# liwanyue123/SRBD-NMPC-Solver

Measured on AMD Instinct MI355X. Metric: SRBD OCP-QP solves/sec (N=20, nx=12, nu=12, fp64) at 1/2/4/8 MI355X, higher is better.
Workload: dtype f64

## Files before the change

srbd-nmpc-solver_amd/csrc/riccati_unconstr_impl.h:

```cpp
namespace srbd {
namespace SRBD_NS {

using real = SRBD_REAL;


struct HbmSrc {
  const ProblemArgsT<real>& a;
  int qp;
  __device__ const real* at(const real* base, int nstage, int blk, int k) const {
    return a.layout == 1 ? base + ((size_t)k * a.batch + qp) * blk
                         : base + ((size_t)qp * nstage + k) * blk;
  }
  __device__ const real* A(int k) const { return at(a.A, a.N, 144, k); }
  __device__ const real* B(int k) const { return at(a.B, a.N, 144, k); }
  __device__ const real* b(int k) const { return at(a.b, a.N, 12, k); }
  __device__ const real* Q(int k) const { return at(a.Q, a.N + 1, 144, k); }
  __device__ const real* S(int k) const { return at(a.S, a.N, 144, k); }
  __device__ const real* R(int k) const { return at(a.R, a.N, 144, k); }
  __device__ const real* q(int k) const { return at(a.q, a.N + 1, 12, k); }
  __device__ const real* r(int k) const { return at(a.r, a.N, 12, k); }
  __device__ real* rec(int k) const { return a.ws + ((size_t)k * a.batch + qp) * kWsStage; }
  real* img = nullptr;
  int gq = 0;
  __device__ real* kept(int k) const { return img + (k * 4 + gq) * kWsStage; }
  template <class StoreRec>
  __device__ void store_stage(int k, StoreRec&& store) const;
};

template <class Src>
constexpr bool keeps_turnaround = std::is_same_v<Src, HbmSrc> && sizeof(real) == 8;

constexpr int kImgA = 0, kImgB = 144, kImgb = 288, kImgQ = 300, kImgS = 444, kImgR = 588,
              kImgq = 732, kImgr = 744, kImgStage = 756, kImgRec = kImgQ;
static_assert(kImgRec + kWsStage <= kImgStage, "a record fits its stage slot past A, B, b");

struct LdsSrc {
  real* img;
  real* grec = nullptr;
  int batch = 0, qp = 0;
  __device__ real* slot(int k) const { return img + k * kImgStage; }
  __device__ const real* A(int k) const { return slot(k) + kImgA; }
  __device__ const real* B(int k) const { return slot(k) + kImgB; }
  __device__ const real* b(int k) const { return slot(k) + kImgb; }
  __device__ const real* Q(int k) const { return slot(k) + kImgQ; }
  __device__ const real* S(int k) const { return slot(k) + kImgS; }
  __device__ const real* R(int k) const { return slot(k) + kImgR; }
  __device__ const real* q(int k) const { return slot(k) + kImgq; }
  __device__ const real* r(int k) const { return slot(k) + kImgr; }
  __device__ real* rec(int k) const {
    return grec ? grec + ((size_t)k * batch + qp) * kWsStage : slot(k) + kImgRec;
  }
};

__device__ __forceinline__ void store_rec_P(real* rec, int lane, const real (&P)[12]) {
  if (lane < kMaxDim) store_packed_col(rec + kWsP, lane, P);
  if (lane == kVecLane) store12(rec + kWsp, P);
}
__device__ __forceinline__ void store_rec(real* rec, int lane, const real (&Kc)[12], const real (&P)[12]) {
  const bool isv = lane == kVecLane;
  if (lane < kMaxDim || isv) {
    const int c = isv ? kMaxDim : lane;
    sfor<0, 12>([&](auto m) {
      constexpr int M = decltype(m)::value;
      rec[kWsK + M * kWsRow + c] = Kc[M];
    });
  }
  store_rec_P(rec, lane, P);
}

constexpr int kRecHotStages = 4;

template <class StoreRec>
__device__ void HbmSrc::store_stage(int k, StoreRec&& store) const {
  if (!img) {
    store(rec(k));
    return;
  }
  if (k < 2) {
    store(kept(k));
    lds_wave_fence();
    return;
  }
  store(img + gq * kWsStage);
  lds_wave_fence();
  const int qp0 = qp - gq;
  const int nq = a.batch - qp0 < 4 ? a.batch - qp0 : 4;
  constexpr int kPiecesPerRec = kWsStage * (int)sizeof(real) / 16;
  const int pieces = nq * kPiecesPerRec;
  typedef double d2 __attribute__((ext_vector_type(2)));
  const d2* src = reinterpret_cast<const d2*>(img);
  d2* dst = reinterpret_cast<d2*>(a.ws + ((size_t)k * a.batch + qp0) * kWsStage);
  const int l = (int)(threadIdx.x & 63);
  if (k >= kRecHotStages) {
    for (int p = l; p < pieces; p += 16 * nq) __builtin_nontemporal_store(src[p], &dst[p]);
  } else {
    for (int p = l; p < pieces; p += 16 * nq) dst[p] = src[p];
  }
  lds_wave_fence();
}

__device__ __forceinline__ void store_riccati_out(const ProblemArgsT<real>& a, int qp, int k, int lane,
                                                  const real (&F)[12], const real (&Kc)[12]) {
  const int N = a.N;
  const bool own = lane < kMaxDim, isv = lane == kVecLane;
  if (a.P && own) store12(a.P + ((size_t)qp * (N + 1) + k) * 144 + (size_t)lane * 12, F);
  if (a.p && isv) store12(a.p + ((size_t)qp * (N + 1) + k) * 12, F);
  if (k < N) {
    if (a.K && own) store12(a.K + ((size_t)qp * N + k) * 144 + (size_t)lane * 12, Kc);
    if (a.k && isv) store12(a.k + ((size_t)qp * N + k) * 12, Kc);
  }
}

constexpr int kLineVec = 4 * 4 * 12;
constexpr int kLineOut = 0;
constexpr int kLineB = 3 * kLineVec;
constexpr int kLinePieces = 4 * 12 * (int)sizeof(real) / 16;
static_assert(kLineB + 2 * kLineVec <= 4 * kWsStage, "the line staging fits slot A");
#ifndef SRBD_RIC_FLUSH_NT
#define SRBD_RIC_FLUSH_NT 1
#endif

template <class Src>
__device__ __forceinline__ void fwd_sweep(const ProblemArgsT<real>& a, const Src& src, const int qp,
                                          const int lane, real* so = nullptr) {
  constexpr int nx = 12, nu = 12;
  const int N = a.N;
  const bool own = lane < kMaxDim;
  const int row = own ? lane : kMaxDim - 1;
  real xv = own ? a.x0[(size_t)qp * nx + lane] : real(0.0);
  bool bad = false;
  real* xo = a.x + (size_t)qp * (N + 1) * nx;
  real* uo = a.u + (size_t)qp * N * nu;
  real* po = a.pi + (size_t)qp * (N + 1) * nx;
  real Pr[12], Kr[12], Ar[12], pv, kv, bv;
  typedef double d2 __attribute__((ext_vector_type(2)));
  typedef __attribute__((address_space(3))) real lds_real;
  typedef __attribute__((address_space(3))) d2 lds_d2;
  lds_real* line = nullptr;
  int gq = 0, qp0 = qp, nq = 1, wl = 0;
  if constexpr (keeps_turnaround<Src>) {
    line = (lds_real*)(uintptr_t)__builtin_amdgcn_readfirstlane((unsigned)(uintptr_t)(lds_real*)src.img);
    gq = src.gq;
    qp0 = __builtin_amdgcn_readfirstlane(qp - gq);
    nq = a.batch - qp0 < 4 ? a.batch - qp0 : 4;
    wl = (int)(threadIdx.x & 63);
  }
  auto piece = [&](int l, int i, int& g, int& w) {
    const int p = l + i * 16 * nq;
    g = p / kLinePieces;
    w = p - g * kLinePieces;
    return p < nq * kLinePieces;
  };
  auto fetch_b = [&](int c) {
    int l = wl;
    opaque(l);
    lds_d2* dst = (lds_d2*)(line + kLineB + (c & 1) * kLineVec);
    d2 bq[2];
    sfor<0, 2>([&](auto i) {
      constexpr int I = decltype(i)::value;
      int g, w;
      bq[I] = d2{0.0, 0.0};
      if (piece(l, I, g, w) && 4 * c + w / 6 < N) {
        const HbmSrc o{a, qp0 + g};
        bq[I] = reinterpret_cast<const d2*>(o.b(4 * c + w / 6))[w % 6];
      }
    });
    sfor<0, 2>([&](auto i) {
      constexpr int I = decltype(i)::value;
      int g, w;
      if (piece(l, I, g, w)) dst[l + I * 16 * nq] = bq[I];
    });
    lds_wave_fence();
  };
  auto flush_out = [&](int c) {
    lds_wave_fence();
    int l = wl;
    opaque(l);
    sfor<0, 2>([&](auto i) {
      constexpr int I = decltype(i)::value;
      int g, w;
      const bool live = piece(l, I, g, w);
      sfor<0, 3>([&](auto v) {
        constexpr int V = decltype(v)::value;
        const int rows = V == 1 ? N : N + 1;
        real* base = V == 0 ? a.x : V == 1 ? a.u : a.pi;
        const int left = rows - 4 * c, nr = left < 4 ? left : 4;
        const lds_d2* from = (const lds_d2*)(line + kLineOut + V * kLineVec);
        if (live && w < 6 * nr) {
          d2* to = reinterpret_cast<d2*>(base + ((size_t)(qp0 + g) * rows + 4 * c) * 12) + w;
          if constexpr (SRBD_RIC_FLUSH_NT) {
            __builtin_nontemporal_store(from[l + I * 16 * nq], to);
          } else {
            *to = from[l + I * 16 * nq];
          }
        }
      });
    });
    lds_wave_fence();
  };
  auto load_rows = [&](int k, real (&P_)[12], real (&K_)[12], real (&A__)[12], real& p_, real& k_,
                       real& b_) {
    const real* rec = src.rec(k);
    load_packed_sym(rec + kWsP, row, P_);
    p_ = rec[kWsp + row];
    if (k < N) {
      const real* kr = rec + kWsK + row * kWsRow;
      const real* Ab = src.A(k);
      sfor<0, 12>([&](auto j) {
        constexpr int J = decltype(j)::value;
        K_[J] = kr[J];
        A__[J] = Ab[J * 12 + row];
      });
      k_ = kr[12];
      if constexpr (keeps_turnaround<Src>) {
        b_ = line[kLineB + ((k >> 2) & 1) * kLineVec + (gq * 4 + (k & 3)) * 12 + row];
      } else {
        b_ = src.b(k)[row];
      }
    }
  };
  auto load_rows_kept = [&](int k, real (&P_)[12], real (&K_)[12], real (&A__)[12], real& p_, real& k_,
                            real& b_) {
    if constexpr (keeps_turnaround<Src>) {
      const auto rec = (const __attribute__((address_space(3))) real*)src.kept(k);
      load_packed_sym(rec + kWsP, row, P_);
      p_ = rec[kWsp + row];
      const auto kr = rec + kWsK + row * kWsRow;
      const real* Ab = src.A(k);
      sfor<0, 12>([&](auto j) {
        constexpr int J = decltype(j)::value;
        K_[J] = kr[J];
        A__[J] = Ab[J * 12 + row];
      });
      k_ = kr[12];
      b_ = src.b(k)[row];
    }
  };
  auto kept = [&](int k) { return keeps_turnaround<Src> && k < 2 && k < N; };
  if (kept(0)) {
    load_rows_kept(0, Pr, Kr, Ar, pv, kv, bv);
    lds_wave_fence();
  } else {
    load_rows(0, Pr, Kr, Ar, pv, kv, bv);
  }
#pragma unroll 1
  for (int k = 0; k <= N; ++k) {
    real Br[12];
    if (k < N) {
      const real* Bb = src.B(k);
      sfor<0, 12>([&](auto j) { Br[decltype(j)::value] = Bb[decltype(j)::value * 12 + row]; });
    }
    const int fc = k == 0 ? 0 : (k >> 2) + 1;
    const bool fetch = keeps_turnaround<Src> && (k == 0 || (k & 3) == 1) && 4 * fc < N;
    real Pn[12], Kn[12], An[12], pvn = real(0.0), kvn = real(0.0), bvn = real(0.0);
    if (k < N) {
      if (kept(k + 1)) {
        load_rows_kept(k + 1, Pn, Kn, An, pvn, kvn, bvn);
      } else {
        load_rows(k + 1, Pn, Kn, An, pvn, kvn, bvn);
      }
    }
    real bx[12];
    sfor<0, 12>([&](auto j) {
      constexpr int J = decltype(j)::value;
      bx[J] = bc<J>(xv);
    });
    real pp = pv;
    sfor<0, 12>([&](auto j) {
      constexpr int J = decltype(j)::value;
      pp = fmadd(Pr[J], bx[J], pp);
    });
    if (own) {
      if constexpr (keeps_turnaround<Src>) {
        line[kLineOut + (gq * 4 + (k & 3)) * 12 + lane] = xv;
        line[kLineOut + 2 * kLineVec + (gq * 4 + (k & 3)) * 12 + lane] = pp;
      } else {
        xo[(size_t)k * nx + lane] = xv;
        po[(size_t)k * nx + lane] = pp;
      }
      if (so) {
        so[k * nx + lane] = xv;
        so[(2 * N + 1) * nx + k * nx + lane] = pp;
      }
    }
    if (k == N) break;
    real uu = kv, xn = bv;
    sfor<0, 12>([&](auto j) {
      constexpr int J = decltype(j)::value;
      uu = fmadd(Kr[J], bx[J], uu);
      xn = fmadd(Ar[J], bx[J], xn);
    });
    if (own) {
      if constexpr (keeps_turnaround<Src>) {
        line[kLineOut + kLineVec + (gq * 4 + (k & 3)) * 12 + lane] = uu;
      } else {
        uo[(size_t)k * nu + lane] = uu;
      }
      if (so) so[(N + 1) * nx + k * nu + lane] = uu;
    }
    xn = dot_bcast(Br, uu, xn);
    bad |= own && (!(uu == uu) || !(xn == xn));
    xv = xn;
    sfor<0, 12>([&](auto j) {
      constexpr int J = decltype(j)::value;
      Pr[J] = Pn[J];
      Kr[J] = Kn[J];
      Ar[J] = An[J];
    });
    pv = pvn;
    kv = kvn;
    bv = bvn;
    if constexpr (keeps_turnaround<Src>) {
      if ((k & 3) == 3) flush_out(k >> 2);
      if (fetch) fetch_b(fc);
    }
  }
  if constexpr (keeps_turnaround<Src>) flush_out(N >> 2);
  if (a.status || a.iter) {
    const unsigned long long m = __ballot(bad);
    const int shift = (threadIdx.x & 63) & ~(kGroup - 1);
    const bool any_bad = ((m >> shift) & 0xffffull) != 0;
    if (lane == 0) {
      if (a.status) a.status[qp] = any_bad ? 3 : 0;
      if (a.iter) a.iter[qp] = 0;
    }
  }
}

template <bool SQRT, class Src>
__device__ __forceinline__ void solve_qp(const ProblemArgsT<real>& a, const Src& src, const int qp,
                                         const int lane, real* so = nullptr) {
  const int N = a.N;
  const bool isv = lane == kVecLane;
  const bool own = lane < kMaxDim;
  const int col = own ? lane : kMaxDim - 1;
  const real reg = a.reg;

  real P[12];
  if (isv) {
    load12(src.q(N), P);
  } else {
    load12(src.Q(N) + col * 12, P);
  }
  store_rec_P(src.rec(N), lane, P);
  store_riccati_out(a, qp, N, lane, P, P);
  if constexpr (SQRT) sqrt_factor(P, lane);

  real A_[12], B_[12];
#pragma unroll 1
  for (int k = N - 1; k >= 0; --k) {
    if (isv) {
      load12(src.b(k), A_);
      sfor<0, 12>([&](auto i) { B_[decltype(i)::value] = real(0.0); });
    } else {
      load12(src.A(k) + col * 12, A_);
      load12(src.B(k) + col * 12, B_);
    }
    auto loadR = [&](real (&Rc)[12]) {
      if (isv) {
        sfor<0, 12>([&](auto i) { Rc[decltype(i)::value] = real(0.0); });
      } else {
        load12(src.R(k) + col * 12, Rc);
      }
    };
    auto loadSQ = [&](real (&Sc)[12], real (&Qc)[12]) {
      if (isv) {
        load12(src.r(k), Sc);
        load12(src.q(k), Qc);
      } else {
        load12(src.S(k) + col * 12, Sc);
        load12(src.Q(k) + col * 12, Qc);
      }
    };
    StageFactor<real> f;
    tstamp(0);
    if constexpr (SQRT) {
      riccati_step_sqrt<1, false>(P, A_, B_, loadR, loadSQ, lane, reg, f);
    } else {
      riccati_step<1, false>(P, A_, B_, loadR, loadSQ, lane, reg, f);
    }
    if constexpr (std::is_same_v<Src, HbmSrc>) {
      src.store_stage(k, [&](real* r) { store_rec(r, lane, f.Kc, f.F); });
    } else {
      store_rec(src.rec(k), lane, f.Kc, f.F);
    }
    tstamp(11);
    store_riccati_out(a, qp, k, lane, f.F, f.Kc);
    sfor<0, 12>([&](auto i) {
      constexpr int I = decltype(i)::value;
      P[I] = f.F[I];
    });
    if constexpr (SQRT) sqrt_factor(P, lane);
  }
  tstamp(12);
  fwd_sweep(a, src, qp, lane, so);
  tstamp(13);
}

template <bool SQRT>
__global__ void __launch_bounds__(256, 2) riccati_unconstr_kernel(ProblemArgsT<real> a) {
  const int gid = blockIdx.x * blockDim.x + threadIdx.x;
  const int qp = gid >> 4;
  if (qp >= a.batch) return;
  if constexpr (sizeof(real) == 8) {
    __shared__ __attribute__((aligned(16))) real rec_img[4 * 2 * 4 * kWsStage];
    static_assert(sizeof(rec_img) <= 64 * 1024, "static LDS limit");
    HbmSrc src{a, qp};
    src.gq = (threadIdx.x >> 4) & 3;
    src.img = rec_img + (threadIdx.x >> 6) * 2 * 4 * kWsStage;
    solve_qp<SQRT>(a, src, qp, threadIdx.x & (kGroup - 1));
  } else {
    solve_qp<SQRT>(a, HbmSrc{a, qp}, qp, threadIdx.x & (kGroup - 1));
  }
}

constexpr int kRealsPerDma = 16 / (int)sizeof(real);
constexpr int kLdsCopyThreads = 512;

__device__ __forceinline__ const real* img_source(const ProblemArgsT<real>& a, int qp, int e) {
  const int N = a.N;
  const int k = e / kImgStage, o = e - k * kImgStage;
  const size_t s = (size_t)qp * N + k, s1 = (size_t)qp * (N + 1) + k;
  if (o >= kImgQ && o < kImgS) return a.Q + s1 * 144 + (o - kImgQ);
  if (o >= kImgq && o < kImgr) return a.q + s1 * 12 + (o - kImgq);
  if (k >= N) return nullptr;
  if (o < kImgB) return a.A + s * 144 + o;
  if (o < kImgb) return a.B + s * 144 + (o - kImgB);
  if (o < kImgQ) return a.b + s * 12 + (o - kImgb);
  if (o < kImgR) return a.S + s * 144 + (o - kImgS);
  if (o < kImgq) return a.R + s * 144 + (o - kImgR);
  return a.r + s * 12 + (o - kImgr);
}

__device__ __forceinline__ void lds_copy_range(const ProblemArgsT<real>& a, real* img, int qp, int e0, int e1,
                                               int t, int nthr) {
  const int wave_off = (t >> 6) * 64 * kRealsPerDma;
  for (int c0 = e0; c0 < e1; c0 += nthr * kRealsPerDma) {
    const int e = c0 + t * kRealsPerDma;
    const real* g = e < e1 ? img_source(a, qp, e) : nullptr;
    if (g)
      __builtin_amdgcn_global_load_lds((const __attribute__((address_space(1))) void*)g,
                                       (__attribute__((address_space(3))) void*)(img + c0 + wave_off), 16,
                                       0, 0);
  }
}
__device__ __forceinline__ void lds_copy_qp(const ProblemArgsT<real>& a, real* img, int qp) {
  lds_copy_range(a, img, qp, 0, (a.N + 1) * kImgStage, threadIdx.x, kLdsCopyThreads);
  tstamp(14);
  asm volatile("s_waitcnt vmcnt(0)" ::: "memory");
  __syncthreads();
  tstamp(15);
}

template <bool SQRT>
__global__ void __launch_bounds__(kLdsCopyThreads, 1) riccati_unconstr_lds_kernel(ProblemArgsT<real> a) {
  extern __shared__ __attribute__((aligned(16))) unsigned char lds_raw[];
  real* img = reinterpret_cast<real*>(lds_raw);
  const int qp = blockIdx.x;
  tstamp(16);
  lds_copy_qp(a, img, qp);
  if (threadIdx.x >= kGroup) return;
  solve_qp<SQRT>(a, LdsSrc{img}, qp, threadIdx.x);
}

size_t lds_image_bytes(int N) { return (size_t)(N + 1) * kImgStage * sizeof(real); }
size_t lds_res_bytes(int N) { return lds_image_bytes(N) + (size_t)(3 * N + 2) * 12 * sizeof(real); }


constexpr int kResThreads = 256;
constexpr int kResStages = kResThreads / 12;
constexpr int kResWavesMax = 8;

__device__ __forceinline__ void max_nan(real& m, real v) {
  v = v < real(0) ? -v : v;
  if (v > m || v != v) m = v;
}

struct ResGlobal {
  const ProblemArgsT<real>& a;
  int qp;
  __device__ const real* at(const real* base, int nstage, size_t blk, int k) const {
    return a.layout == 1 ? base + ((size_t)k * a.batch + qp) * blk : base + ((size_t)qp * nstage + k) * blk;
  }
  __device__ const real* A(int k) const { return at(a.A, a.N, (size_t)a.nx * a.nx, k); }
  __device__ const real* B(int k) const { return at(a.B, a.N, (size_t)a.nx * a.nu, k); }
  __device__ const real* b(int k) const { return at(a.b, a.N, a.nx, k); }
  __device__ const real* Q(int k) const { return at(a.Q, a.N + 1, (size_t)a.nx * a.nx, k); }
  __device__ const real* S(int k) const { return at(a.S, a.N, (size_t)a.nx * a.nu, k); }
  __device__ const real* R(int k) const { return at(a.R, a.N, (size_t)a.nu * a.nu, k); }
  __device__ const real* q(int k) const { return at(a.q, a.N + 1, a.nx, k); }
  __device__ const real* r(int k) const { return at(a.r, a.N, a.nu, k); }
  __device__ const real* x() const { return a.x + (size_t)qp * (a.N + 1) * a.nx; }
  __device__ const real* u() const { return a.u + (size_t)qp * a.N * a.nu; }
  __device__ const real* pi() const { return a.pi + (size_t)qp * (a.N + 1) * a.nx; }
};
struct ResLds : LdsSrc {
  const real* so;
  int N;
  __device__ const real* x() const { return so; }
  __device__ const real* u() const { return so + (N + 1) * 12; }
  __device__ const real* pi() const { return so + (2 * N + 1) * 12; }
};

template <class Acc, int DIM = 0>
__device__ __forceinline__ void unconstr_residuals_body(const ProblemArgsT<real>& a, const Acc& acc, int qp, int t) {
  const int N = a.N, nx = DIM ? DIM : a.nx, nu = DIM ? DIM : a.nu;
  if (a.stat) {
    real* tab = a.stat + (size_t)qp * a.stat_rows * kStatCols;
    for (int i = t; i < a.stat_rows * kStatCols; i += blockDim.x) tab[i] = real(0);
  }
  const real* x = acc.x();
  const real* u = acc.u();
  const real* pi = acc.pi();
  const int i = t % 12;
  real mg = real(0), mb = real(0), ob = real(0);
  for (int k = t / 12; t < kResStages * 12 && k <= N; k += kResStages) {
    const real* xk = x + (size_t)k * nx;
    if (k < N) {
      const real* uk = u + (size_t)k * nu;
      const real* xn = x + (size_t)(k + 1) * nx;
      const real* pn = pi + (size_t)(k + 1) * nx;
      const real* A = acc.A(k);
      const real* B = acc.B(k);
      if (i < nu) {
        const real* S = acc.S(k);
        const real* R = acc.R(k);
        const real* r = acc.r(k);
        real ru = real(0), sx = real(0), bp = real(0);
        for (int j = 0; j < nu; ++j) ru += R[(size_t)j * nu + i] * uk[j];
        for (int j = 0; j < nx; ++j) sx += S[(size_t)j * nu + i] * xk[j];
        for (int j = 0; j < nx; ++j) bp += B[(size_t)i * nx + j] * pn[j];
        max_nan(mg, ru + sx + r[i] + bp);
        ob += uk[i] * (real(0.5) * ru + r[i] + sx);
      }
      if (i < nx) {
        const real* b = acc.b(k);
        real v = b[i] - xn[i];
        for (int j = 0; j < nx; ++j) v += A[(size_t)j * nx + i] * xk[j];
        for (int j = 0; j < nu; ++j) v += B[(size_t)j * nx + i] * uk[j];
        max_nan(mb, v);
      }
    }
    if (k > 0 && i < nx) {
      const real* Q = acc.Q(k);
      const real* q = acc.q(k);
      real qx = real(0), g = q[i] - pi[(size_t)k * nx + i];
      for (int j = 0; j < nx; ++j) qx += Q[(size_t)j * nx + i] * xk[j];
      g += qx;
      if (k < N) {
        const real* uk = u + (size_t)k * nu;
        const real* pn = pi + (size_t)(k + 1) * nx;
        const real* A = acc.A(k);
        const real* S = acc.S(k);
        for (int j = 0; j < nu; ++j) g += S[(size_t)i * nu + j] * uk[j];
        for (int j = 0; j < nx; ++j) g += A[(size_t)i * nx + j] * pn[j];
      }
      max_nan(mg, g);
      ob += xk[i] * (real(0.5) * qx + q[i]);
    }
  }
  for (int m = 32; m >= 1; m >>= 1) {
    const real og = __shfl_xor(mg, m), obb = __shfl_xor(mb, m);
    if (og > mg || og != og) mg = og;
    if (obb > mb || obb != obb) mb = obb;
    ob += __shfl_xor(ob, m);
  }
  __shared__ real part[3][kResWavesMax];
  const int w = t / 64;
  if ((t & 63) == 0) {
    part[0][w] = mg;
    part[1][w] = mb;
    part[2][w] = ob;
  }
  __syncthreads();
  if (t == 0) {
    mg = part[0][0], mb = part[1][0], ob = part[2][0];
    for (int j = 1; j < kResThreads / 64; ++j) {
      if (part[0][j] > mg || part[0][j] != part[0][j]) mg = part[0][j];
      if (part[1][j] > mb || part[1][j] != part[1][j]) mb = part[1][j];
      ob += part[2][j];
    }
    if (a.res) {
      a.res[(size_t)qp * 4 + 0] = mg;
      a.res[(size_t)qp * 4 + 1] = mb;
      a.res[(size_t)qp * 4 + 2] = real(0);
      a.res[(size_t)qp * 4 + 3] = real(0);
    }
    if (a.obj) a.obj[qp] = ob;
    if (a.stat) {
      real* row = a.stat + (size_t)qp * a.stat_rows * kStatCols;
      row[6] = mg;
      row[7] = mb;
      row[10] = ob;
    }
    if (a.status && (mg != mg || mb != mb)) a.status[qp] = 3;
  }
}

__global__ void __launch_bounds__(kResThreads) unconstr_residuals_kernel(ProblemArgsT<real> a) {
  unconstr_residuals_body(a, ResGlobal{a, (int)blockIdx.x}, (int)blockIdx.x, (int)threadIdx.x);
}

template <bool SQRT>
__global__ void __launch_bounds__(kLdsCopyThreads, 1) riccati_unconstr_lds_res_kernel(ProblemArgsT<real> a) {
  extern __shared__ __attribute__((aligned(16))) unsigned char lds_raw[];
  real* img = reinterpret_cast<real*>(lds_raw);
  real* so = img + (a.N + 1) * kImgStage;
  const int qp = blockIdx.x;
  tstamp(16);
  lds_copy_qp(a, img, qp);
  LdsSrc src{img};
  src.grec = a.ws;
  src.batch = a.batch;
  src.qp = qp;
  if (threadIdx.x < kGroup) solve_qp<SQRT>(a, src, qp, threadIdx.x, so);
  __syncthreads();
  ResLds acc{};
  acc.img = img;
  acc.so = so;
  acc.N = a.N;
  unconstr_residuals_body(a, acc, qp, (int)threadIdx.x);
}

template <bool FULL>
__global__ void __launch_bounds__(256) unconstr_residuals_group_kernel(ProblemArgsT<real> a) {
  __shared__ __attribute__((aligned(16))) real tb_all[(256 / kGroup) * 144];
  const int qp = (int)((blockIdx.x * blockDim.x + threadIdx.x) >> 4);
  const int lane = threadIdx.x & (kGroup - 1);
  if (qp >= a.batch) return;
  real* const tb = tb_all + (threadIdx.x >> 4) * 144;
  const int N = a.N, nx = FULL ? 12 : a.nx, nu = FULL ? 12 : a.nu;
  if (a.stat) {
    real* tab = a.stat + (size_t)qp * a.stat_rows * kStatCols;
    for (int i = lane; i < a.stat_rows * kStatCols; i += kGroup) tab[i] = real(0);
  }
  const bool smaj = a.layout == 1;
  auto at = [&](const real* base, int nstage, size_t blk, int k) -> const real* {
    return smaj ? base + ((size_t)k * a.batch + qp) * blk : base + ((size_t)qp * nstage + k) * blk;
  };
  const size_t nxx = (size_t)nx * nx, nxu = (size_t)nx * nu, nuu = (size_t)nu * nu;
  const real* x = a.x + (size_t)qp * (N + 1) * nx;
  const real* u = a.u + (size_t)qp * N * nu;
  const real* pi = a.pi + (size_t)qp * (N + 1) * nx;
  const int li = lane < kMaxDim ? lane : 0;
  const bool xl = lane < nx, ul = lane < nu;
  auto colv = [&](const real* blk, int rows, int cols, real (&v)[12]) {
    if constexpr (FULL) {
      load12(blk + li * 12, v);
    } else {
      load_col_pad(blk + (size_t)li * rows, rows, lane < cols, v);
    }
  };
  auto row_sum = [&](const real (&T)[12]) -> real {
    lds_wave_fence();
    if (lane < kMaxDim) store12(tb + lane * 12, T);
    lds_wave_fence();
    real s = real(0);
    sfor<0, 12>([&](auto j) { s += tb[decltype(j)::value * 12 + li]; });
    return s;
  };
  real mg = real(0), mb = real(0), ob = real(0);
#pragma unroll 1
  for (int k = 0; k <= N; ++k) {
    const real xk = xl ? x[(size_t)k * nx + lane] : real(0);
    real T[12];
    real gx = real(0);
    if (k > 0) {
      real Qc[12];
      colv(at(a.Q, N + 1, nxx, k), nx, nx, Qc);
      sfor<0, 12>([&](auto i) { T[decltype(i)::value] = Qc[decltype(i)::value] * xk; });
      const real qx = row_sum(T);
      const real qk = xl ? at(a.q, N + 1, nx, k)[lane] : real(0);
      gx = qx + qk - (xl ? pi[(size_t)k * nx + lane] : real(0));
      if (xl) ob += xk * (real(0.5) * qx + qk);
    }
    if (k < N) {
      const real uk = ul ? u[(size_t)k * nu + lane] : real(0);
      const real xn = xl ? x[(size_t)(k + 1) * nx + lane] : real(0);
      const real pin = xl ? pi[(size_t)(k + 1) * nx + lane] : real(0);
      real Ac[12], Bc[12];
      colv(at(a.A, N, nxx, k), nx, nx, Ac);
      colv(at(a.B, N, nxu, k), nx, nu, Bc);
      const real atp = dot_bcast(Ac, pin, real(0));
      const real btp = dot_bcast(Bc, pin, real(0));
      sfor<0, 12>([&](auto i) {
        constexpr int I = decltype(i)::value;
        T[I] = fmadd(Ac[I], xk, Bc[I] * uk);
      });
      const real axbu = row_sum(T);
      if (xl) max_nan(mb, axbu + at(a.b, N, nx, k)[lane] - xn);
      real Sc[12], Rc[12];
      colv(at(a.S, N, nxu, k), nu, nx, Sc);
      colv(at(a.R, N, nuu, k), nu, nu, Rc);
      const real stu = dot_bcast(Sc, uk, real(0));
      sfor<0, 12>([&](auto i) {
        constexpr int I = decltype(i)::value;
        T[I] = fmadd(Rc[I], uk, Sc[I] * xk);
      });
      const real rusx = row_sum(T);
      const real rk = ul ? at(a.r, N, nu, k)[lane] : real(0);
      if (ul) {
        max_nan(mg, rusx + rk + btp);
        ob += uk * (real(0.5) * rusx + rk);
      }
      if (xl) ob += real(0.5) * xk * stu;
      gx += stu + atp;
    }
    if (k > 0 && xl) max_nan(mg, gx);
  }
  sfor<0, 4>([&](auto s) {
    constexpr int M = 8 >> decltype(s)::value;
    const real og = __shfl_xor(mg, M, kGroup), obb = __shfl_xor(mb, M, kGroup);
    if (og > mg || og != og) mg = og;
    if (obb > mb || obb != obb) mb = obb;
    ob += __shfl_xor(ob, M, kGroup);
  });
  if (lane == 0) {
    if (a.res) {
      a.res[(size_t)qp * 4 + 0] = mg;
      a.res[(size_t)qp * 4 + 1] = mb;
      a.res[(size_t)qp * 4 + 2] = real(0);
      a.res[(size_t)qp * 4 + 3] = real(0);
    }
    if (a.obj) a.obj[qp] = ob;
    if (a.stat) {
      real* row = a.stat + (size_t)qp * a.stat_rows * kStatCols;
      row[6] = mg;
      row[7] = mb;
      row[10] = ob;
    }
    if (a.status && (mg != mg || mb != mb)) a.status[qp] = 3;
  }
}

constexpr int kResGroupMin = 256;

hipError_t launch_residuals(const ProblemArgsT<real>& a, hipStream_t stream) {
  if (a.batch <= 0) return hipSuccess;
  if (a.batch <= kResGroupMin) {
    hipLaunchKernelGGL(unconstr_residuals_kernel, dim3((unsigned)a.batch), dim3(kResThreads), 0, stream, a);
    return hipGetLastError();
  }
  const unsigned blocks = (unsigned)(((long long)a.batch * kGroup + 255) / 256);
  if (a.nx == 12 && a.nu == 12) {
    hipLaunchKernelGGL(unconstr_residuals_group_kernel<true>, dim3(blocks), dim3(256), 0, stream, a);
  } else {
    hipLaunchKernelGGL(unconstr_residuals_group_kernel<false>, dim3(blocks), dim3(256), 0, stream, a);
  }
  return hipGetLastError();
}

constexpr int kLdsBatchMax = 256;
constexpr size_t kLdsBytesMax = 160 * 1024;
constexpr size_t kLdsResStatic = 1024;

bool use_lds_kernel(const ProblemArgsT<real>& a) {
  return a.layout == 0 && a.batch <= kLdsBatchMax && lds_image_bytes(a.N) <= kLdsBytesMax;
}

#if SRBD_WITH_LATENCY
#include "riccati_latency_impl.h"
bool lat_eligible(const ProblemArgsT<real>& a) { return use_lds_kernel(a) && lat_fits(a.N); }
#else
bool lat_eligible(const ProblemArgsT<real>&) { return false; }
#endif

bool fused_residuals(const ProblemArgsT<real>& a) {
  return a.fuse_res && (a.res || a.obj || a.stat) && a.nx == 12 && a.nu == 12 && use_lds_kernel(a) &&
         lds_res_bytes(a.N) + kLdsResStatic <= kLdsBytesMax;
}
bool reads_once(const ProblemArgsT<real>& a) {
  return a.nx == 12 && a.nu == 12 && use_lds_kernel(a) &&
         (fused_residuals(a) || !(a.res || a.obj || a.stat));
}

template <bool SQRT>
static hipError_t launch_alg(const ProblemArgsT<real>& a, hipStream_t stream) {
#if SRBD_WITH_LATENCY
  if (!SQRT && lat_eligible(a)) {
    if (fused_residuals(a)) {
      hipLaunchKernelGGL(riccati_latency_kernel<true>, dim3((unsigned)a.batch), dim3(kLatThreads),
                         lat_lds_bytes(a.N), stream, a);
    } else {
      hipLaunchKernelGGL(riccati_latency_kernel<false>, dim3((unsigned)a.batch), dim3(kLatThreads),
                         lat_lds_bytes(a.N), stream, a);
    }
    return hipGetLastError();
  }
#endif
  if (fused_residuals(a)) {
    hipLaunchKernelGGL(riccati_unconstr_lds_res_kernel<SQRT>, dim3((unsigned)a.batch), dim3(kLdsCopyThreads),
                       lds_res_bytes(a.N), stream, a);
    return hipGetLastError();
  }
  if (use_lds_kernel(a)) {
    const size_t bytes = lds_image_bytes(a.N);
    hipLaunchKernelGGL(riccati_unconstr_lds_kernel<SQRT>, dim3((unsigned)a.batch), dim3(kLdsCopyThreads), bytes,
                       stream, a);
    return hipGetLastError();
  }
  const int threads = 256;
  const long long lanes = (long long)a.batch * kGroup;
  const int blocks = (int)((lanes + threads - 1) / threads);
  hipLaunchKernelGGL(riccati_unconstr_kernel<SQRT>, dim3(blocks), dim3(threads), 0, stream, a);
  return hipGetLastError();
}

#if SRBD_WITH_LATENCY
bool server_ok(const ProblemArgsT<real>& a) {
  return a.batch == 1 && !a.ric_alg && lat_eligible(a) && reads_once(a);
}
hipError_t launch_server(const ProblemArgsT<real>& a, LatMailbox* mb, int epoch, int last_done,
                         long long idle_ticks, long long life_ticks, hipStream_t stream) {
  if (!server_ok(a)) return hipErrorInvalidValue;
  if (fused_residuals(a))
    hipLaunchKernelGGL(riccati_latency_server_kernel<true>, dim3(1), dim3(kLatThreads), lat_lds_bytes(a.N), stream,
                       a, mb, epoch, last_done, idle_ticks, life_ticks);
  else
    hipLaunchKernelGGL(riccati_latency_server_kernel<false>, dim3(1), dim3(kLatThreads), lat_lds_bytes(a.N), stream,
                       a, mb, epoch, last_done, idle_ticks, life_ticks);
  return hipGetLastError();
}
#endif

hipError_t prepare_device() {
  hipError_t e = hipFuncSetAttribute(reinterpret_cast<const void*>(&riccati_unconstr_lds_kernel<false>),
                                     hipFuncAttributeMaxDynamicSharedMemorySize, (int)kLdsBytesMax);
  if (e == hipSuccess)
    e = hipFuncSetAttribute(reinterpret_cast<const void*>(&riccati_unconstr_lds_kernel<true>),
                            hipFuncAttributeMaxDynamicSharedMemorySize, (int)kLdsBytesMax);
  if (e == hipSuccess)
    e = hipFuncSetAttribute(reinterpret_cast<const void*>(&riccati_unconstr_lds_res_kernel<false>),
                            hipFuncAttributeMaxDynamicSharedMemorySize, (int)(kLdsBytesMax - kLdsResStatic));
  if (e == hipSuccess)
    e = hipFuncSetAttribute(reinterpret_cast<const void*>(&riccati_unconstr_lds_res_kernel<true>),
                            hipFuncAttributeMaxDynamicSharedMemorySize, (int)(kLdsBytesMax - kLdsResStatic));
#if SRBD_WITH_LATENCY
  if (e == hipSuccess)
    e = hipFuncSetAttribute(reinterpret_cast<const void*>(&riccati_latency_kernel<false>),
                            hipFuncAttributeMaxDynamicSharedMemorySize, (int)(kLdsBytesMax - kLdsResStatic));
  if (e == hipSuccess)
    e = hipFuncSetAttribute(reinterpret_cast<const void*>(&riccati_latency_kernel<true>),
                            hipFuncAttributeMaxDynamicSharedMemorySize, (int)(kLdsBytesMax - kLdsResStatic));
  if (e == hipSuccess)
    e = hipFuncSetAttribute(reinterpret_cast<const void*>(&riccati_latency_server_kernel<false>),
                            hipFuncAttributeMaxDynamicSharedMemorySize, (int)(kLdsBytesMax - kLdsResStatic));
  if (e == hipSuccess)
    e = hipFuncSetAttribute(reinterpret_cast<const void*>(&riccati_latency_server_kernel<true>),
                            hipFuncAttributeMaxDynamicSharedMemorySize, (int)(kLdsBytesMax - kLdsResStatic));
#endif
  return e;
}

hipError_t launch(const ProblemArgsT<real>& a, hipStream_t stream) {
  if (a.batch <= 0) return hipSuccess;
  if (a.nx != 12 || a.nu != 12) return hipErrorInvalidValue;
  return a.ric_alg ? launch_alg<true>(a, stream) : launch_alg<false>(a, stream);
}

}
}
```

Measured before the change: 21.85 million.

## Keep stage-0 Riccati factors in registers and compute u0, pi0 directly

In the fp64 LDS turnaround path, the backward sweep now keeps the stage-0 gain and cost-to-go in registers instead of writing a record to LDS. The forward sweep computes u0 and pi0 straight from those registers with cross-lane broadcasts. The kept LDS slots move to stages 1 and 2, and the line staging buffer shifts to the second half of the image. The stage-2 b value is read from the staged line buffer. This removes a record store, a fence and a reload at the turnaround, at the cost of extra broadcast arithmetic and higher register pressure.

```diff
diff --git a/srbd-nmpc-solver_amd/csrc/riccati_unconstr_impl.h b/srbd-nmpc-solver_amd/csrc/riccati_unconstr_impl.h
--- a/srbd-nmpc-solver_amd/csrc/riccati_unconstr_impl.h
+++ b/srbd-nmpc-solver_amd/csrc/riccati_unconstr_impl.h
@@ -22,7 +22,7 @@
   __device__ real* rec(int k) const { return a.ws + ((size_t)k * a.batch + qp) * kWsStage; }
   real* img = nullptr;
   int gq = 0;
-  __device__ real* kept(int k) const { return img + (k * 4 + gq) * kWsStage; }
+  __device__ real* kept(int k) const { return img + ((k == 1 ? 4 : 0) + gq) * kWsStage; }
   template <class StoreRec>
   __device__ void store_stage(int k, StoreRec&& store) const;
 };
@@ -76,7 +76,8 @@
     store(rec(k));
     return;
   }
-  if (k < 2) {
+  if (k == 0) return;
+  if (k <= 2) {
     store(kept(k));
     lds_wave_fence();
     return;
@@ -115,14 +116,48 @@
 constexpr int kLineOut = 0;
 constexpr int kLineB = 3 * kLineVec;
 constexpr int kLinePieces = 4 * 12 * (int)sizeof(real) / 16;
-static_assert(kLineB + 2 * kLineVec <= 4 * kWsStage, "the line staging fits slot A");
+static_assert(kLineB + 2 * kLineVec <= 4 * kWsStage, "the line staging fits slot B");
 #ifndef SRBD_RIC_FLUSH_NT
 #define SRBD_RIC_FLUSH_NT 1
 #endif
 
+__device__ __forceinline__ void stage0_u_pi(const real x0, const real (&Kc)[12], const real (&F)[12],
+                                            const int row, real& u0, real& pi0) {
+  real bx[12], acc[12];
+  sfor<0, 12>([&](auto j) { bx[decltype(j)::value] = bc<decltype(j)::value>(x0); });
+  auto own_entry = [&]() {
+    real v = acc[0];
+    sfor<1, 12>([&](auto i) {
+      v = row == decltype(i)::value ? acc[decltype(i)::value] : v;
+      opaque(v);
+    });
+    return v;
+  };
+  sfor<0, 12>([&](auto i) { acc[decltype(i)::value] = bc<kVecLane>(Kc[decltype(i)::value]); });
+  sfor<0, 12>([&](auto j) {
+    constexpr int J = decltype(j)::value;
+    fma_bcast_src<J>(acc, Kc, bx[J]);
+  });
+  u0 = own_entry();
+  sfor<0, 12>([&](auto i) { acc[decltype(i)::value] = bc<kVecLane>(F[decltype(i)::value]); });
+  sfor<0, 12>([&](auto j) {
+    constexpr int J = decltype(j)::value;
+    sfor<0, 12>([&](auto i) {
+      constexpr int I = decltype(i)::value;
+      if constexpr (J <= I) {
+        acc[I] = fmadd(bc<J>(F[I]), bx[J], acc[I]);
+      } else {
+        acc[I] = fmadd(bc<I>(F[J]), bx[J], acc[I]);
+      }
+    });
+  });
+  pi0 = own_entry();
+}
+
 template <class Src>
 __device__ __forceinline__ void fwd_sweep(const ProblemArgsT<real>& a, const Src& src, const int qp,
-                                          const int lane, real* so = nullptr) {
+                                          const int lane, real* so = nullptr,
+                                          const real (*K0)[12] = nullptr, const real (*P0)[12] = nullptr) {
   constexpr int nx = 12, nu = 12;
   const int N = a.N;
   const bool own = lane < kMaxDim;
@@ -139,7 +174,8 @@
   lds_real* line = nullptr;
   int gq = 0, qp0 = qp, nq = 1, wl = 0;
   if constexpr (keeps_turnaround<Src>) {
-    line = (lds_real*)(uintptr_t)__builtin_amdgcn_readfirstlane((unsigned)(uintptr_t)(lds_real*)src.img);
+    line = (lds_real*)(uintptr_t)__builtin_amdgcn_readfirstlane(
+        (unsigned)(uintptr_t)(lds_real*)(src.img + 4 * kWsStage));
     gq = src.gq;
     qp0 = __builtin_amdgcn_readfirstlane(qp - gq);
     nq = a.batch - qp0 < 4 ? a.batch - qp0 : 4;
@@ -233,13 +269,19 @@
         A__[J] = Ab[J * 12 + row];
       });
       k_ = kr[12];
-      b_ = src.b(k)[row];
+      if (k == 2) {
+        b_ = line[kLineB + (gq * 4 + 2) * 12 + row];
+      } else {
+        b_ = src.b(k)[row];
+      }
     }
   };
-  auto kept = [&](int k) { return keeps_turnaround<Src> && k < 2 && k < N; };
-  if (kept(0)) {
-    load_rows_kept(0, Pr, Kr, Ar, pv, kv, bv);
-    lds_wave_fence();
+  auto kept = [&](int k) { return keeps_turnaround<Src> && (k == 1 || k == 2) && k < N; };
+  if constexpr (keeps_turnaround<Src>) {
+    const real* Ab = src.A(0);
+    sfor<0, 12>([&](auto j) { Ar[decltype(j)::value] = Ab[decltype(j)::value * 12 + row]; });
+    bv = src.b(0)[row];
+    stage0_u_pi(xv, *K0, *P0, row, kv, pv);
   } else {
     load_rows(0, Pr, Kr, Ar, pv, kv, bv);
   }
@@ -256,6 +298,7 @@
     if (k < N) {
       if (kept(k + 1)) {
         load_rows_kept(k + 1, Pn, Kn, An, pvn, kvn, bvn);
+        lds_wave_fence();
       } else {
         load_rows(k + 1, Pn, Kn, An, pvn, kvn, bvn);
       }
@@ -265,11 +308,14 @@
       constexpr int J = decltype(j)::value;
       bx[J] = bc<J>(xv);
     });
+    const bool given = keeps_turnaround<Src> && k == 0;
     real pp = pv;
-    sfor<0, 12>([&](auto j) {
-      constexpr int J = decltype(j)::value;
-      pp = fmadd(Pr[J], bx[J], pp);
-    });
+    if (!given) {
+      sfor<0, 12>([&](auto j) {
+        constexpr int J = decltype(j)::value;
+        pp = fmadd(Pr[J], bx[J], pp);
+      });
+    }
     if (own) {
       if constexpr (keeps_turnaround<Src>) {
         line[kLineOut + (gq * 4 + (k & 3)) * 12 + lane] = xv;
@@ -285,11 +331,24 @@
     }
     if (k == N) break;
     real uu = kv, xn = bv;
-    sfor<0, 12>([&](auto j) {
-      constexpr int J = decltype(j)::value;
-      uu = fmadd(Kr[J], bx[J], uu);
-      xn = fmadd(Ar[J], bx[J], xn);
-    });
+    if constexpr (keeps_turnaround<Src>) {
+      if (!given) {
+        sfor<0, 12>([&](auto j) {
+          constexpr int J = decltype(j)::value;
+          uu = fmadd(Kr[J], bx[J], uu);
+        });
+      }
+      sfor<0, 12>([&](auto j) {
+        constexpr int J = decltype(j)::value;
+        xn = fmadd(Ar[J], bx[J], xn);
+      });
+    } else {
+      sfor<0, 12>([&](auto j) {
+        constexpr int J = decltype(j)::value;
+        uu = fmadd(Kr[J], bx[J], uu);
+        xn = fmadd(Ar[J], bx[J], xn);
+      });
+    }
     if (own) {
       if constexpr (keeps_turnaround<Src>) {
         line[kLineOut + kLineVec + (gq * 4 + (k & 3)) * 12 + lane] = uu;
@@ -347,6 +406,7 @@
   if constexpr (SQRT) sqrt_factor(P, lane);
 
   real A_[12], B_[12];
+  [[maybe_unused]] real K0[12];
 #pragma unroll 1
   for (int k = N - 1; k >= 0; --k) {
     if (isv) {
@@ -390,10 +450,20 @@
       constexpr int I = decltype(i)::value;
       P[I] = f.F[I];
     });
+    if constexpr (keeps_turnaround<Src>) {
+      if (k == 0) {
+        sfor<0, 12>([&](auto i) { K0[decltype(i)::value] = f.Kc[decltype(i)::value]; });
+        break;
+      }
+    }
     if constexpr (SQRT) sqrt_factor(P, lane);
   }
   tstamp(12);
-  fwd_sweep(a, src, qp, lane, so);
+  if constexpr (keeps_turnaround<Src>) {
+    fwd_sweep(a, src, qp, lane, so, &K0, &P);
+  } else {
+    fwd_sweep(a, src, qp, lane, so);
+  }
   tstamp(13);
 }
 
```

Result: no change. 22.01 million (median of 6 runs) (+0.8%).
